# kjyv/FloBaRoID

Measured on AMD Instinct MI355X. Metric: regressor samples/s (fused regressor->Gram pass) + TSQR TFLOP/s, WALK-MAN 31-DOF float-base, higher is better.
Workload: dtype f64

## Files before the change

### flobaroid_amd/csrc/fbr_gram64.h

```cpp
#pragma once
#define FBR_G64_SWZ(c) (2 * ((c) & 15))
#include <algorithm>
#include <type_traits>
#include <utility>

#include "fbr_kinid.h"

struct FbrGram64 {
    int NT = 0;
    int NF = 0;
    int nlev = 0, fb = 0, flev = 0, ntr = 0, maxact = 0, npw = 0, wpb = 8;
    long blk_doubles = 0;
    std::vector<int> trow;
    std::vector<int> slab;
    int nstage = 0, base_stages = 0;
    std::vector<int> stage_lev;
    std::vector<int> lev_begin;
    std::vector<int> pieces;
    std::vector<int> wmeta;
    std::vector<int> slot_tiles;
    std::vector<int> tilecol;
    std::vector<int> fcol_tile, fcol_slot;
    std::vector<int> tile_lo;
    long mfma_per_block = 0;
    long busiest = 0, balanced = 0;
};

static inline bool fbr_gram64_build(const FbrHostModel &hm, const FbrGramProgram &gp, FbrGram64 &g, bool force_tiles = true, bool wide16 = false)
{
    if (gp.T != 1 || (gp.k > 0 && gp.rhs_tiles)) return false;
    g.npw = gp.cfg.segw * gp.cfg.nseg;
    g.wpb = FBR_WPB;
    if (wide16 && g.npw > 10) {
        g.wpb = 2 * FBR_WPB;
        g.npw = 10;
    }
    const int W = g.wpb;
    g.NT = gp.NT;
    g.fb = hm.fb;
    g.nlev = 0;
    std::vector<int> tlo(gp.NT, 0), thi(gp.NT, 0);
    for (int t = 0; t < gp.NT; t++) {
        const FbrTile &tl = gp.tiles[t];
        if (tl.type != 0) return false;
        thi[t] = hm.fb + (int)tl.tpath.size();
        if (tl.friction) {
            int jmin = (int)tl.tpath.size(), jmax = -1;
            for (int sl = 0; sl < FBR_TILE; sl++) {
                if (tl.col[sl] < 0) continue;
                const int jnt = hm.coldesc[tl.col[sl]].joint;
                for (int j = 0; j < (int)tl.tpath.size(); j++)
                    if (tl.tpath[j] == jnt) jmin = std::min(jmin, j), jmax = std::max(jmax, j);
// ... 147 lines not shown
                const int w1 = wave_of[i];
                if (w2 == w1 || cnt[w2] >= g.npw) continue;
                shift(i, w1, -1), shift(i, w2, +1);
                long c1, q1;
                score(c1, q1);
                if (c1 < c0 || (c1 == c0 && q1 < q0)) {
                    wave_of[i] = w2, c0 = c1, q0 = q1, improved = 1;
                } else {
                    shift(i, w2, -1), shift(i, w1, +1);
                }
            }
            for (int k2 = i + 1; k2 < NP; k2++) {
                const int w1 = wave_of[i], w2 = wave_of[k2];
                if (w1 == w2 || (prs[i].lo == prs[k2].lo && prs[i].hi == prs[k2].hi)) continue;
                shift(i, w1, -1), shift(k2, w2, -1), shift(i, w2, +1), shift(k2, w1, +1);
                long c1, q1;
                score(c1, q1);
                if (c1 < c0 || (c1 == c0 && q1 < q0)) {
                    wave_of[i] = w2, wave_of[k2] = w1, c0 = c1, q0 = q1, improved = 1;
                } else {
                    shift(i, w2, -1), shift(k2, w1, -1), shift(i, w1, +1), shift(k2, w2, +1);
                }
            }
        }
    }
    g.busiest = c0;
    g.balanced = 0;
    for (int sg = 0; sg < g.nstage; sg++) {
        int tot = 0;
        for (int lv = g.stage_lev[sg]; lv < g.stage_lev[sg + 1]; lv++)
            for (int w = 0; w < W; w++) tot += wl[w][lv];
        g.balanced += (tot + W - 1) / W;
    }
    g.wmeta.assign((size_t)W * g.npw * 3, -1);
    g.slot_tiles.assign((size_t)2 * W * g.npw * 2, -1);
    g.mfma_per_block = 0;
    for (int w = 0; w < W; w++) {
        std::vector<int> mine;
        for (int i = 0; i < NP; i++)
            if (wave_of[i] == w) mine.push_back(i);
        std::vector<char> done(NP, 0);
        int q = 0;
        for (size_t left = mine.size(); left > 0;) {
            std::vector<int> freq(NTT, 0);
            for (int i : mine)
                if (!done[i]) {
                    freq[prs[i].a]++;
                    if (prs[i].b != prs[i].a) freq[prs[i].b]++;
                }
            int T = 0;
            for (int t = 1; t < NTT; t++)
                if (freq[t] > freq[T]) T = t;
            for (int i : mine) {
                if (done[i] || (prs[i].a != T && prs[i].b != T)) continue;
                const int J = prs[i].a == T ? prs[i].b : prs[i].a;
                const size_t s = (size_t)w * g.npw + q;
                const size_t sr = ((size_t)(w & 7) * (W / 8) + (size_t)(w >> 3)) * g.npw + q;
                g.wmeta[3 * s] = T;
                g.wmeta[3 * s + 1] = J;
                g.wmeta[3 * s + 2] = prs[i].lo | (prs[i].hi << 8);
                const int kind = T >= g.NT ? 1 : 0;
                g.slot_tiles[((size_t)kind * W * g.npw + sr) * 2] = T;
                g.slot_tiles[((size_t)kind * W * g.npw + sr) * 2 + 1] = J;
                g.mfma_per_block += 16L * (prs[i].hi - prs[i].lo);
                done[i] = 1;
                q++;
                left--;
            }
        }
    }
    return true;
}

#define FBR_G64_WORDS 18
#define FBR_G64_FRIC 4
struct FbrGram64Producer {
    int nparts = 1, nslots = 1, step0[FBR_KINWRITE_PARTS] = {0, 0, 0, 0}, nsteps[FBR_KINWRITE_PARTS] = {0, 0, 0, 0};
    std::vector<long long> rel;
    std::vector<int> lcol;
    std::vector<int> steps;
};

static inline bool fbr_gram64_build_producer(const FbrHostModel &hm, const FbrGramProgram &gp, const FbrGram64 &g, FbrGram64Producer &pr)
{
    std::vector<int> tile_of(hm.cols, -1), slot_of(hm.cols, -1);
    for (int t = 0; t < g.NT; t++)
        for (int sl = 0; sl < FBR_TILE; sl++)
            if (gp.tiles[t].col[sl] >= 0 && gp.tiles[t].col[sl] < hm.cols) {
                tile_of[gp.tiles[t].col[sl]] = t;
                slot_of[gp.tiles[t].col[sl]] = sl;
            }
    std::vector<double> lcost(hm.L, 30.0);
    for (int c = 0; c < hm.ninert; c++)
        if (tile_of[c] >= 0) lcost[hm.coldesc[c].link] += 10.0 + (double)(hm.fb + hm.path[hm.coldesc[c].link].size());
    std::vector<FbrKinIdProgram> progs;
    std::vector<std::vector<char>> own;
    try {
        fbr_kinid_build_parts(hm, lcost, FBR_KINWRITE_PARTS, progs, own);
    } catch (const std::exception &) {
        return false;
    }
    pr.nparts = (int)progs.size();
    pr.rel.assign((size_t)pr.nparts * FBR_G64_WORDS * hm.L, 0);
    pr.lcol.assign((size_t)pr.nparts * (10 + FBR_G64_FRIC) * hm.L, -1);
// ... 20 lines not shown
    for (int c = hm.ninert; c < hm.cols; c++) {
        const int t = tile_of[c], sl = slot_of[c], d = hm.coldesc[c].joint, p = (c - hm.ninert) / std::max(hm.n, 1);
        if (t < 0) continue;
        int l = -1;
        for (int x = 0; x < hm.L; x++)
            if (hm.dof[x] == d) l = x;
        if (l < 0 || p >= FBR_G64_FRIC || hm.path[l].empty() || hm.path[l].back() != d) return false;
        const int lv = hm.fb + (int)hm.path[l].size() - 1;
        if (lv < g.tile_lo[t] || g.trow[(size_t)t * g.nlev + lv] < 0) return false;
        const long long tr0 = (long long)g.trow[(size_t)t * g.nlev + g.tile_lo[t]] - g.tile_lo[t];
        if (tr0 < 0) return false;
        for (int pq = 0; pq < pr.nparts; pq++)
            if (own[pq][l]) {
                pr.rel[((size_t)pq * hm.L + l) * FBR_G64_WORDS + 14 + p] = word(tr0, sl);
                pr.lcol[(size_t)pr.nparts * 10 * hm.L + ((size_t)pq * hm.L + l) * FBR_G64_FRIC + p] = c;
            }
    }
    pr.steps.clear();
    pr.nslots = 1;
    for (int pq = 0; pq < pr.nparts; pq++) {
        pr.step0[pq] = (int)(pr.steps.size() / FBR_KINID_STEP);
        pr.nsteps[pq] = progs[pq].nsteps;
        pr.nslots = std::max(pr.nslots, progs[pq].nslots);
        pr.steps.insert(pr.steps.end(), progs[pq].steps.begin(), progs[pq].steps.begin() + (size_t)progs[pq].nsteps * FBR_KINID_STEP);
    }
    return true;
}

#if defined(__HIPCC__) && defined(FBR_KERNELS_GRAM)
struct DevGram64 {
    int NT, nlev, maxact, npieces, nstage;
    long blk_doubles;
    const int *slab, *lev_begin, *pieces, *wmeta, *stage_lev;
};

template <int MAXD, bool HASW>
__global__ __launch_bounds__(64 * FBR_KINWRITE_PARTS, MAXD <= 10 ? 2 : 1) void fbr_kinimg_kernel(DevModel m, DevKinId p, DevKinWrite wr, long S, long blk_doubles,
                                                                              const double *__restrict__ q, const double *__restrict__ dq,
                                                                              const double *__restrict__ ddq, const double *__restrict__ bv,
                                                                              const double *__restrict__ ba, const double *__restrict__ rpy,
                                                                              const double *__restrict__ rhs, const double *__restrict__ wts,
                                                                              double *__restrict__ scratch, double *__restrict__ mom,
                                                                              const double *__restrict__ sign)
{
    extern __shared__ __attribute__((aligned(16))) double smem[];
    const int lane = threadIdx.x & 63, part = __builtin_amdgcn_readfirstlane(threadIdx.x >> 6), nth = blockDim.x, tid = threadIdx.x;
    const int n = m.n, ldn = p.ldn, ldw = m.rows | 1, rows = m.rows;
    double *sq = smem, *sdq = sq + 64 * ldn, *sddq = sdq + 64 * ldn, *sw = sddq + 64 * ldn;
    double *st = sw + (HASW ? 64 * ldw : 0);
    double *scr = scratch + ((long)blockIdx.x * wr.nparts + part) * p.nslots * FBR_LINK_REC * 64 + lane;
    double *mo = mom ? mom + (long)blockIdx.x * (wr.cols + 1) * 64 : nullptr;
    const long Sg = wr.group_samples > 0 ? wr.group_samples : S, bpg = (Sg + 63) >> 6;
    const long nblk = (S / Sg) * bpg;
    const fbr_clong_ptr cdst = (fbr_clong_ptr)(unsigned long)wr.dst;
    const fbr_cint_ptr ccol = (fbr_cint_ptr)(unsigned long)(wr.lcol10 + (long)part * 10 * m.L);
    for (long blk = blockIdx.x; blk < nblk; blk += gridDim.x) {
        const long grp = blk / bpg, lb = blk - grp * bpg;
        const long base = grp * Sg + (lb << 6);
        const int valid = (int)min(64L, Sg - (lb << 6));
        __syncthreads();
        {
            const long off = base * n;
            const int cnt = valid * n;
            int sr = tid / n, dc = tid - sr * n;
            const int ds = nth / n, dd = nth - ds * n;
            for (int i = tid; i < cnt; i += nth) {
// ... 189 lines not shown
        blk[(long)tr * 1024 + (sl >> 5) * 512 + c * 32 + ((sl & 31) ^ FBR_G64_SWZ(c))] = 0.0;
    }
}

__global__ __launch_bounds__(256) void fbr_gram64_mom_reduce_kernel(int P, int nwg, const double *__restrict__ mom, double *__restrict__ G)
{
    __shared__ double part[256];
    const int c = blockIdx.x, t = threadIdx.x;
    double s0 = 0.0, s1 = 0.0, s2 = 0.0, s3 = 0.0;
    int i = t;
    for (; i + 768 < nwg * 64; i += 1024) {
        s0 += mom[((long)(i >> 6) * (P + 1) + c) * 64 + (i & 63)];
        s1 += mom[((long)((i + 256) >> 6) * (P + 1) + c) * 64 + ((i + 256) & 63)];
        s2 += mom[((long)((i + 512) >> 6) * (P + 1) + c) * 64 + ((i + 512) & 63)];
        s3 += mom[((long)((i + 768) >> 6) * (P + 1) + c) * 64 + ((i + 768) & 63)];
    }
    for (; i < nwg * 64; i += 256) s0 += mom[((long)(i >> 6) * (P + 1) + c) * 64 + (i & 63)];
    part[t] = (s0 + s1) + (s2 + s3);
    __syncthreads();
    for (int o = 128; o > 0; o >>= 1) {
        if (t < o) part[t] += part[t + o];
        __syncthreads();
    }
    if (t) return;
    const int Pa = P + 1;
    if (c == P) {
        G[(long)P * Pa + P] += part[0];
    } else {
        G[(long)c * Pa + P] += part[0];
        G[(long)P * Pa + c] += part[0];
    }
}

template <int NPW, int WPB>
__global__ __launch_bounds__(WPB * 64, (NPW <= 10) ? 4 : 2) void fbr_gram64_kernel(DevGram64 g, long nblk, const double *__restrict__ img,
                                                                                  double *__restrict__ partial, int carry)
{
    constexpr int MW = 3 * NPW;
    static_assert(MW <= 64, "a wave's slot table is fetched with one load");
    extern __shared__ __attribute__((aligned(16))) double smem[];
    const int bufd = g.maxact * 512;
    double *buf0 = smem, *buf1 = smem + bufd;
    int *slab = (int *)(smem + 2 * bufd);
    int *levb = slab + g.nlev * g.NT;
    int *pcs = levb + g.nlev + 1;
    int *wm = pcs + 2 * g.npieces;
    int *stl = wm + WPB * MW;
    const int tid = threadIdx.x, lane = tid & 63;
    const int wave = __builtin_amdgcn_readfirstlane(tid >> 6);
    for (int i = tid; i < g.nlev * g.NT; i += WPB * 64) slab[i] = g.slab[i];
    for (int i = tid; i <= g.nlev; i += WPB * 64) levb[i] = g.lev_begin[i];
    for (int i = tid; i < 2 * g.npieces; i += WPB * 64) pcs[i] = g.pieces[i];
    for (int i = tid; i < WPB * MW; i += WPB * 64) wm[i] = g.wmeta[i];
    for (int i = tid; i <= g.nstage; i += WPB * 64) stl[i] = g.stage_lev[i];
    fbr_d4 acc[NPW];
    img += (long)blockIdx.y * nblk * g.blk_doubles;
    double *pp = partial + (((((long)blockIdx.y * gridDim.x + blockIdx.x) * 8 + (wave & 7)) * (WPB / 8) + (wave >> 3)) * NPW) * 256;
    if (carry) {
#pragma unroll
        for (int q = 0; q < NPW; q++) acc[q] = (fbr_d4){pp[q * 256 + lane], pp[q * 256 + 64 + lane], pp[q * 256 + 128 + lane], pp[q * 256 + 192 + lane]};
    } else {
#pragma unroll
        for (int q = 0; q < NPW; q++) acc[q] = (fbr_d4){0.0, 0.0, 0.0, 0.0};
    }
    __syncthreads();
    const int nmine = (int)((nblk - blockIdx.x + gridDim.x - 1) / gridDim.x);
    const long nst = (long)(nmine > 0 ? nmine : 0) * 2 * g.nstage;
    const int svl = stl[lane <= g.nstage ? lane : 0], svp = levb[svl];
    auto dma = [&](int sg, long bh, int par) {
        const long blk = (long)blockIdx.x + (bh >> 1) * gridDim.x;
        const double *src = img + blk * g.blk_doubles + (bh & 1) * 512 + 2 * lane;
        double *buf = par ? buf1 : buf0;
        const int i0 = __builtin_amdgcn_readlane(svp, sg) + wave, i1 = __builtin_amdgcn_readlane(svp, sg + 1);
        const int mine = i0 < i1 ? (i1 - i0 + WPB - 1) / WPB : 0;
        const int il = i0 + (lane < mine ? lane : 0) * WPB;
        const int gxv = mine > 0 ? pcs[2 * il] : 0, lxv = mine > 0 ? pcs[2 * il + 1] : 0;
        for (int j = 0; j < mine; j++) {
            const int gx = __builtin_amdgcn_readlane(gxv, j), lx = __builtin_amdgcn_readlane(lxv, j);
            __builtin_amdgcn_global_load_lds((fbr_glb_ptr)(src + gx), (fbr_lds_ptr)(buf + lx), 16, 0, 0);
        }
    };
    if (nst > 0) dma(0, 0, 0);
    const int li = lane & 15, kk = lane >> 4;
    const int lofs = li * 32, sx = FBR_G64_SWZ(li);
    const int mv = wm[wave * MW + (lane < MW ? lane : 0)];
    const int idxv = (lane < MW && (lane % 3) != 2 && mv >= 0) ? mv : 0;
    const int p0c = lofs | (sx ^ kk);
    int sg = 0;
    long bh = 0;
    for (long st = 0; st < nst; st++) {
        asm volatile("s_waitcnt vmcnt(0)" ::: "memory");
        __syncthreads();
        const int sgn = sg + 1 == g.nstage ? 0 : sg + 1;
        const long bhn = sgn ? bh : bh + 1;
        if (st + 1 < nst) dma(sgn, bhn, (int)((st + 1) & 1));
        const double *buf = (st & 1) ? buf1 : buf0;
        const int lv0 = __builtin_amdgcn_readlane(svl, sg), lv1 = __builtin_amdgcn_readlane(svl, sg + 1);
        sg = sgn;
        bh = bhn;
        for (int lv = lv0; lv < lv1; lv++) {
            const int offv = slab[lv * g.NT + idxv] * 512;
            int curI = -1;
            double a[8] = {0.0, 0.0, 0.0, 0.0, 0.0, 0.0, 0.0, 0.0};
#pragma unroll
            for (int q = 0; q < NPW; q++) {
                const int tI = __builtin_amdgcn_readlane(mv, 3 * q), rg = __builtin_amdgcn_readlane(mv, 3 * q + 2);
                if (tI < 0 || lv < (rg & 0xff) || lv >= (rg >> 8)) continue;
                const double *pb = buf + __builtin_amdgcn_readlane(offv, 3 * q + 1);
                double b[NPW <= 10 ? 4 : 8];
                int p0 = p0c;
                if constexpr (NPW <= 10) asm volatile("" : "+v"(p0));
                if (tI != curI) {
                    const double *pa = buf + __builtin_amdgcn_readlane(offv, 3 * q);
#pragma unroll
                    for (int ks = 0; ks < 8; ks++) a[ks] = pa[p0 ^ (4 * ks)];
                    curI = tI;
                }
                constexpr int KG = NPW <= 10 ? 4 : 8;
#pragma unroll
                for (int k0 = 0; k0 < 8; k0 += KG) {
#pragma unroll
                    for (int ks = k0; ks < k0 + KG; ks++) b[ks - k0] = pb[p0 ^ (4 * ks)];
                    __builtin_amdgcn_sched_barrier(0);
#pragma unroll
                    for (int ks = k0; ks < k0 + KG; ks++) acc[q] = __builtin_amdgcn_mfma_f64_16x16x4f64(a[ks], b[ks - k0], acc[q], 0, 0, 0);
                    __builtin_amdgcn_sched_barrier(0);
                }
            }
        }
    }
#pragma unroll
    for (int q = 0; q < NPW; q++) {
        pp[q * 256 + 0 * 64 + lane] = acc[q][0];
        pp[q * 256 + 1 * 64 + lane] = acc[q][1];
        pp[q * 256 + 2 * 64 + lane] = acc[q][2];
        pp[q * 256 + 3 * 64 + lane] = acc[q][3];
    }
}
#endif
```

### flobaroid_amd/csrc/fbr_gram_api.hip

```cpp
#define FBR_KERNELS_GRAM
#include "fbr_internal.h"

static int get_deal(GramHolder *h, int wpg, GramHolder::Deal *out, bool base_only = false)
{
    const int key = wpg | (base_only ? 1 << 24 : 0);
    auto it = h->deals.find(key);
    if (it != h->deals.end()) {
        *out = it->second;
        return FBR_OK;
    }
    const std::vector<int> n = fbr_gram_deal(h->prog, wpg, base_only);
    std::vector<int2> tab;
    std::vector<int> begin(h->prog.T + 1, 0), given(h->prog.T, 0);
    for (int p = 0; p < h->prog.T; p++) begin[p + 1] = begin[p] + n[p];
    while ((int)tab.size() < begin[h->prog.T])
        for (int p = 0; p < h->prog.T; p++)
            if (given[p] < n[p]) tab.push_back(make_int2(p, given[p]++ | (n[p] << 16)));
    GramHolder::Deal d;
    int rc;
    if ((rc = upload(h->pool, tab, &d.tab))) return rc;
    if ((rc = upload(h->pool, begin, &d.begin))) return rc;
    h->deals[key] = d;
    *out = d;
    return FBR_OK;
// ... 174 lines not shown
    if (num_pairs) *num_pairs = (int32_t)h->prog.pairs.size();
    if (mfma_per_sample) *mfma_per_sample = h->prog.mfma_per_sample;
    if (num_parts) *num_parts = h->prog.T;
    return FBR_OK;
}

static int get_gram64(fbr_model *m, GramHolder *h);

extern "C" int fbr_gram_lane_info(const fbr_model *mc, int32_t k, int64_t num_samples, int64_t info[12])
{
    if (!mc || !info) {
        set_err("null model / info");
        return FBR_E_INVALID;
    }
    fbr_model *m = const_cast<fbr_model *>(mc);
    if (int rc_enter = enter(m)) return rc_enter;
    if (const int wr = pick_gram_reduction(m, num_samples < 0 ? -1 : (long)num_samples); wr >= 0) m = m->rdm[wr].get();
    for (int i = 0; i < 12; i++) info[i] = 0;
    if ((m->hm.rows + 3) / 4 * 4 > 60) return FBR_OK;
    const bool moments = fbr_gram_rhs_moments(m->hm, k, m->opt.gram_rhs_tile != 0);
    GramHolder *h = nullptr;
    int rc = get_gram(m, k, &h, moments);
    if (rc) return rc;
    if (!m->opt.gram_lane || k > 1 || (k == 1 && !moments)) return FBR_OK;
    if ((rc = get_gram64(m, h))) return rc;
    if (h->g64_state != 1) return FBR_OK;
    const FbrGram64 &g = h->g64;
    info[0] = 1;
    info[1] = g.ntr;
    info[2] = g.blk_doubles * (int64_t)sizeof(double);
    info[3] = g.mfma_per_block;
    info[4] = g.nlev;
    info[5] = g.maxact;
    info[6] = (int64_t)((size_t)2 * g.maxact * 512 * sizeof(double) +
                        ((size_t)g.nlev * (g.NT + g.NF) + g.nlev + 1 + g.pieces.size() + g.wmeta.size() + g.stage_lev.size()) * sizeof(int));
    info[7] = g.NT;
    info[8] = g.NF;
    info[9] = g.busiest;
    info[10] = g.balanced;
    info[11] = g.nstage;
    return FBR_OK;
}

__global__ __launch_bounds__(256) void fbr_rtr_kernel(int Pa, const double *__restrict__ R, double *__restrict__ G, int accumulate)
{
    for (long e = (long)blockIdx.x * blockDim.x + threadIdx.x; e < (long)Pa * Pa; e += (long)gridDim.x * blockDim.x) {
        const int i = (int)(e / Pa), j = (int)(e % Pa);
        double acc = 0.0;
        for (int r = 0; r <= min(i, j); r++) acc += R[(long)r * Pa + i] * R[(long)r * Pa + j];
        G[e] = accumulate ? G[e] + acc : acc;
    }
}

static int gram_via_tsqr(fbr_model *m, const fbr_states *st, const double *rhs, int32_t k, const double *w, double *G_out, int32_t out_mem,
                         int32_t accumulate)
{
    const int Pa = m->hm.cols + k;
    const size_t cnt = (size_t)Pa * Pa;
    int rc;
    if ((rc = m->gram_r_tmp.ensure(cnt * sizeof(double)))) return rc;
    double *R = m->gram_r_tmp.as<double>();
    if ((rc = tsqr_impl(m, st, nullptr, 0, rhs, k, w, nullptr, R, FBR_DEVICE, nullptr))) return rc;
    double *G = G_out;
    if (out_mem == FBR_HOST) {
        if ((rc = m->g_tmp.ensure(cnt * sizeof(double)))) return rc;
        G = m->g_tmp.as<double>();
        if (accumulate) HIPCHK(hipMemcpyAsync(G, G_out, cnt * sizeof(double), hipMemcpyHostToDevice, m->stream));
    }
    hipLaunchKernelGGL(fbr_rtr_kernel, dim3(1024), dim3(256), 0, m->stream, Pa, R, G, accumulate ? 1 : 0);
    HIPCHK(hipGetLastError());
    return finish_output(m, G, G_out, cnt, out_mem);
}
static int get_gram64(fbr_model *m, GramHolder *h)
{
    if (h->g64_state) return FBR_OK;
    h->g64_state = -1;
    const FbrHostModel &hm = m->hm;
    if (m->kinid.nsteps <= 0 || !fbr_gram64_build(hm, h->prog, h->g64, m->opt.gram_force_tiles != 0, m->opt.gram_lane_waves >= 16)) return FBR_OK;
    FbrGram64 &g = h->g64;
    const size_t lds = (size_t)2 * g.maxact * 512 * sizeof(double) +
                       ((size_t)g.nlev * (g.NT + g.NF) + g.nlev + 1 + g.pieces.size() + g.wmeta.size() + g.stage_lev.size()) * sizeof(int);
    if (lds > 156 * 1024) return FBR_OK;
    const size_t plds_max = ((size_t)3 * 64 * (std::max(hm.n, 1) | 1) + (size_t)2 * 64 * (hm.rows | 1)) * sizeof(double);
    if (plds_max > 160 * 1024) return FBR_OK;
    if (!fbr_gram64_build_producer(hm, h->prog, g, h->g64p)) return FBR_OK;
    std::vector<int> wgbegin{0, 0};
    int rc;
    if ((rc = upload(h->pool, g.slab, &h->d64_slab)) || (rc = upload(h->pool, g.lev_begin, &h->d64_levb)) || (rc = upload(h->pool, g.pieces, &h->d64_pieces)) ||
        (rc = upload(h->pool, g.wmeta, &h->d64_wmeta)) || (rc = upload(h->pool, h->g64p.lcol, &h->d64_lcol)) ||
        (rc = upload(h->pool, h->g64p.steps, &h->d64_steps)) ||
        (rc = upload(h->pool, g.slot_tiles, &h->d64_slot_tiles)) || (rc = upload(h->pool, g.tilecol, &h->d64_tilecol)) ||
        (rc = upload(h->pool, g.stage_lev, &h->d64_stagelev)))
        return rc;
    h->g64_state = 1;
    return FBR_OK;
}

static long gram64_chunk_blocks(const FbrGram64 &g) { return std::max<long>(1, (long)((size_t)3 * 1024 * 1024 * 1024 / ((size_t)g.blk_doubles * 8))); }

static int gram64_wg_table(GramHolder *h, int wgs, const int **out)
{
    auto it = h->d64_wb.find(wgs);
    if (it == h->d64_wb.end()) {
        std::vector<int> wb{0, wgs};
        const int *dwb = nullptr;
        if (int rc = upload(h->pool, wb, &dwb)) return rc;
        it = h->d64_wb.emplace(wgs, dwb).first;
    }
    *out = it->second;
    return FBR_OK;
}

static int gram64_ensure_images(fbr_model *m, GramHolder *h, long chb)
{
    const FbrGram64 &g = h->g64;
    int rc;
    if (chb <= h->img64_blocks) return FBR_OK;
    for (int b = 0; b < 2; b++) {
        if ((rc = h->img64[b].ensure((size_t)chb * g.blk_doubles * sizeof(double)))) return rc;
        HIPCHK(hipMemsetAsync(h->img64[b].p, 0, h->img64[b].bytes, m->stream));
        std::vector<long long> dst(h->g64p.rel.size(), 0);
        for (size_t i = 0; i < dst.size(); i++)
            if (h->g64p.rel[i]) dst[i] = (long long)(uintptr_t)h->img64[b].p + (h->g64p.rel[i] & ~(1LL << 62));
        if ((rc = h->dst64[b].ensure(dst.size() * sizeof(long long)))) return rc;
        HIPCHK(hipMemcpyAsync(h->dst64[b].p, dst.data(), dst.size() * sizeof(long long), hipMemcpyHostToDevice, m->stream));
        HIPCHK(hipStreamSynchronize(m->stream));
    }
    h->img64_blocks = chb;
    return FBR_OK;
}

static int gram64_pass(fbr_model *m, GramHolder *h, const DevStates &d, const double *drhs, const double *dw, int k, double *G, bool base_only,
                       bool h2d_chunked)
{
    const FbrHostModel &hm = m->hm;
    FbrGram64 &g = h->g64;
    const long S = d.S;
    const int Pa = hm.cols + k;
    int rc;
    const long nblocks = (S + 63) / 64;
    long chb = gram64_chunk_blocks(g);
    if (h2d_chunked) chb = std::min<long>(chb, 7L * m->num_cus);
    if (m->opt.chunk_samples >= 1) chb = std::min(gram64_chunk_blocks(g), std::max<long>(1, ((long)m->opt.chunk_samples + 63) / 64));
    chb = std::min(nblocks, chb);
    if (chb < nblocks && chb > m->num_cus) chb = chb / m->num_cus * m->num_cus;
    if ((rc = gram64_ensure_images(m, h, chb))) return rc;
    const int ldn = std::max(hm.n, 1) | 1, ldw = hm.rows | 1;
    const size_t plds = ((size_t)3 * 64 * ldn + (dw ? (size_t)64 * ldw : 0) + (k ? (size_t)64 * ldw : 0)) * sizeof(double);
    const int pgrid_max = (m->kinid.maxlvl <= 10 ? 2 : 1) * m->num_cus;
    const int pblocks = (int)std::min<long>(chb, (long)pgrid_max);
    const int gwgs = (int)std::min<long>(chb, (long)m->num_cus);
    if ((rc = h->scr64.ensure((size_t)pgrid_max * h->g64p.nparts * std::max(h->g64p.nslots, 1) * FBR_LINK_REC * 64 * sizeof(double)))) return rc;
    if (k) {
        if ((rc = h->mom64.ensure((size_t)pgrid_max * (hm.cols + 1) * 64 * sizeof(double)))) return rc;
        HIPCHK(hipMemsetAsync(h->mom64.p, 0, (size_t)pblocks * (hm.cols + 1) * 64 * sizeof(double), m->stream));
    }
    const int npw = g.npw;
    if ((rc = m->partial.ensure((size_t)m->num_cus * g.wpb * npw * 256 * sizeof(double)))) return rc;
    const size_t glds = (size_t)2 * g.maxact * 512 * sizeof(double) + ((size_t)g.nlev * (g.NT + g.NF) + g.nlev + 1 + g.pieces.size() + g.wmeta.size() + g.stage_lev.size()) * sizeof(int);
    DevKinId kp;
    kp.nsteps = 0;
    kp.maxlvl = m->kinid.maxlvl;
    kp.nslots = h->g64p.nslots;
    kp.ldn = ldn;
    kp.steps = h->d64_steps;
    kp.endflush = m->kinid_endflush;
    DevGram64 dg;
    dg.NT = g.NT + g.NF;
    dg.nlev = g.nlev;
    dg.maxact = g.maxact;
    dg.npieces = (int)g.pieces.size() / 2;
    dg.blk_doubles = g.blk_doubles;
    dg.slab = h->d64_slab;
    dg.lev_begin = h->d64_levb;
    dg.pieces = h->d64_pieces;
    dg.wmeta = h->d64_wmeta;
    dg.nstage = base_only ? g.base_stages : g.nstage;
    dg.stage_lev = h->d64_stagelev;
    typedef void (*g64_fn)(DevGram64, long, const double *, double *, int);
    const g64_fn gk = g.wpb == 16 ? fbr_gram64_kernel<10, 16> : (g.npw == 10 ? fbr_gram64_kernel<10, 8> : fbr_gram64_kernel<FBR_ONE_SEGW * FBR_ONE_NSEG, 8>);
    const int vnpw = g.npw * (g.wpb / 8);
    HIPCHK(hipFuncSetAttribute((const void *)gk, hipFuncAttributeMaxDynamicSharedMemorySize, (int)glds));
    int launches = 0, first_wgs = 0;
    const size_t stage_per = (size_t)3 * hm.n + (hm.floating ? 15 : 0) + (d.sign ? hm.n : 0) + (size_t)hm.rows * k + (dw ? hm.rows : 0);
    if (h2d_chunked) {
        for (int b = 0; b < 2; b++)
            if ((rc = m->st_chunk[b].ensure(std::max<size_t>(1, (size_t)chb * 64 * stage_per) * sizeof(double)))) return rc;
        if (!m->copy) {
            int least = 0, greatest = 0;
            HIPCHK(hipDeviceGetStreamPriorityRange(&least, &greatest));
            HIPCHK(hipStreamCreateWithPriority(&m->copy, hipStreamNonBlocking, greatest));
        }
        HIPCHK(hipEventRecord(m->ev_fork, m->stream));
    }
    struct Staged {
        DevStates dc;
        long o;
        const double *rhs, *w;
    };
    auto stage = [&](long c, Staged &out) -> int {
        const long s0 = c * chb * 64, cs = std::min(chb * 64, S - s0);
        const int b = (int)(c & 1);
        out.dc = d;
        out.o = s0;
        out.rhs = drhs;
        out.w = dw;
        if (!h2d_chunked) return FBR_OK;
        HIPCHK(hipStreamWaitEvent(m->copy, m->ev_pack_rec[b] ? m->ev_pack[b] : m->ev_fork, 0));
        ProfScope ps(m, FBR_PROF_H2D, m->copy);
        double *p = m->st_chunk[b].as<double>();
        auto put = [&](const double *src, size_t per, const double **dst) -> int {
            *dst = nullptr;
            if (!src || per == 0) return FBR_OK;
// ... 97 lines not shown
        if ((rc = gram64_wg_table(h, first_wgs, &dr.wg_begin))) return rc;
        dr.tilecol = h->d64_tilecol;
        hipLaunchKernelGGL(fbr_gram_reduce_kernel, dim3(FBR_WPB * vnpw, 1), dim3(256), 0, m->stream, dr, m->partial.as<double>(), G);
        HIPCHK(hipGetLastError());
        if (g.NF > 0) {
            dr.slot_tiles = h->d64_slot_tiles + (size_t)FBR_WPB * vnpw * 2;
            hipLaunchKernelGGL(fbr_gram_reduce_kernel, dim3(FBR_WPB * vnpw, 1), dim3(256), 0, m->stream, dr, m->partial.as<double>(), G);
            HIPCHK(hipGetLastError());
        }
        if (k) {
            hipLaunchKernelGGL(fbr_gram64_mom_reduce_kernel, dim3(hm.cols + 1), dim3(256), 0, m->stream, hm.cols, pblocks, h->mom64.as<double>(), G);
            HIPCHK(hipGetLastError());
        }
    }
    (void)Pa;
    return FBR_OK;
}

static int gram64_grouped_pass(fbr_model *m, GramHolder *h, const DevStates &d, const double *dw, double *G, int ngroups)
{
    const FbrHostModel &hm = m->hm;
    FbrGram64 &g = h->g64;
    const long S = d.S, Sg = S / ngroups, bpg = (Sg + 63) / 64;
    const int Pa = hm.cols, npw = g.npw;
    int rc;
    const int gpc = (int)std::min<long>(std::min(ngroups, 32768), std::max<long>(1, gram64_chunk_blocks(g) / bpg));
    if ((rc = gram64_ensure_images(m, h, (long)gpc * bpg))) return rc;
    const int wpg = (int)std::max<long>(1, std::min<long>(bpg, (long)m->num_cus / std::min(gpc, ngroups)));
    const int ldn = std::max(hm.n, 1) | 1, ldw = hm.rows | 1;
    const size_t plds = ((size_t)3 * 64 * ldn + (dw ? (size_t)64 * ldw : 0)) * sizeof(double);
    const int pgrid_max = (m->kinid.maxlvl <= 10 ? 2 : 1) * m->num_cus;
    if ((rc = h->scr64.ensure((size_t)pgrid_max * h->g64p.nparts * std::max(h->g64p.nslots, 1) * FBR_LINK_REC * 64 * sizeof(double)))) return rc;
    if ((rc = m->partial.ensure((size_t)gpc * wpg * g.wpb * npw * 256 * sizeof(double)))) return rc;
    const size_t glds = (size_t)2 * g.maxact * 512 * sizeof(double) + ((size_t)g.nlev * (g.NT + g.NF) + g.nlev + 1 + g.pieces.size() + g.wmeta.size() + g.stage_lev.size()) * sizeof(int);
    DevKinId kp;
    kp.nsteps = 0;
    kp.maxlvl = m->kinid.maxlvl;
    kp.nslots = h->g64p.nslots;
    kp.ldn = ldn;
    kp.steps = h->d64_steps;
    kp.endflush = m->kinid_endflush;
    DevGram64 dg;
    dg.NT = g.NT + g.NF;
    dg.nlev = g.nlev;
    dg.maxact = g.maxact;
    dg.npieces = (int)g.pieces.size() / 2;
    dg.blk_doubles = g.blk_doubles;
    dg.slab = h->d64_slab;
    dg.lev_begin = h->d64_levb;
    dg.pieces = h->d64_pieces;
    dg.wmeta = h->d64_wmeta;
    dg.nstage = g.nstage;
    dg.stage_lev = h->d64_stagelev;
    typedef void (*g64_fn)(DevGram64, long, const double *, double *, int);
    const g64_fn gk = g.wpb == 16 ? fbr_gram64_kernel<10, 16> : (g.npw == 10 ? fbr_gram64_kernel<10, 8> : fbr_gram64_kernel<FBR_ONE_SEGW * FBR_ONE_NSEG, 8>);
    const int vnpw = g.npw * (g.wpb / 8);
    HIPCHK(hipFuncSetAttribute((const void *)gk, hipFuncAttributeMaxDynamicSharedMemorySize, (int)glds));
    const int *wgb = nullptr;
    if ((rc = gram64_wg_table(h, wpg, &wgb))) return rc;
    int launches = 0;
    for (int g0 = 0; g0 < ngroups; g0 += gpc, launches++) {
        const int ng = std::min(gpc, ngroups - g0), b = launches & 1;
        const long s0 = (long)g0 * Sg, cs = (long)ng * Sg, nb = (long)ng * bpg;
        DevKinWrite kw;
        kw.lcol10 = h->d64_lcol;
        kw.colrec = nullptr;
        kw.dst = (const long *)h->dst64[b].p;
        kw.ninert = hm.ninert;
        kw.cols = hm.cols;
        kw.k = 0;
        kw.has_w = dw ? 1 : 0;
        kw.flev = g.flev;
        kw.base_only = 0;
        kw.group_samples = Sg;
        kw.nparts = h->g64p.nparts;
        for (int pq = 0; pq < FBR_KINWRITE_PARTS; pq++) {
            kw.part_nsteps[pq] = h->g64p.nsteps[pq];
            kw.part_step0[pq] = h->g64p.step0[pq];
        }
        const int pblocks = (int)std::min<long>(nb, (long)pgrid_max);
        if (Sg & 63) {
            hipLaunchKernelGGL(fbr_gram64_tail_zero_kernel, dim3(16, ng), dim3(256), 0, m->stream, h->img64[b].as<double>(), g.blk_doubles, bpg, g.ntr, (int)(Sg & 63));
            HIPCHK(hipGetLastError());
        }
        {
            ProfScope ps(m, FBR_PROF_PACK);
#define FBR_KINIMG_GLAUNCH2(D, W)                                                                                                                 \
    do {                                                                                                                                         \
// ... 456 lines not shown
```

### flobaroid_amd/csrc/fbr_internal.h

```cpp
#pragma once
#include <hip/hip_runtime.h>
#include <unistd.h>

#include <algorithm>
#include <cstdint>
#include <cstdio>
#include <cstdlib>
#include <cstring>
#include <map>
#include <memory>
#include <numeric>
#include <string>
#include <vector>

#include "../../include/fbr.h"
#include "fbr_options.h"
#include "fbr_kernels.h"
#include "fbr_kinid.h"
#include "fbr_gram64.h"
#include "fbr_tsqr_work.h"

extern thread_local std::string g_fbr_err;
static inline void set_err(const std::string &s) { g_fbr_err = s; }

// ... 49 lines not shown
        p = nullptr;
        bytes = 0;
    }
    template <class T> T *as() { return (T *)p; }
};

template <class T> static inline int upload(std::vector<DevBuf> &pool, const std::vector<T> &v, const T **out)
{
    pool.emplace_back();
    DevBuf &b = pool.back();
    size_t n = std::max<size_t>(v.size(), 1) * sizeof(T);
    int rc = b.ensure(n);
    if (rc) return rc;
    if (!v.empty()) HIPCHK(hipMemcpy(b.p, v.data(), v.size() * sizeof(T), hipMemcpyHostToDevice));
    *out = (const T *)b.p;
    return FBR_OK;
}

struct GramHolder {
    FbrGramProgram prog;
    DevGram dev;
    std::vector<DevBuf> pool;
    DevBuf pimg[2];
    bool moments = false;
    DevBuf mom[2];
    bool mom_clean[2] = {false, false};
    const int *itemcol = nullptr;
    size_t lds_bytes = 0;
    size_t pack_lds_bytes = 0;
    int g64_state = 0;
    FbrGram64 g64;
    FbrGram64Producer g64p;
    const int *d64_slab = nullptr, *d64_levb = nullptr, *d64_pieces = nullptr, *d64_wmeta = nullptr, *d64_lcol = nullptr,
              *d64_steps = nullptr, *d64_slot_tiles = nullptr, *d64_tilecol = nullptr, *d64_stagelev = nullptr;
    DevBuf img64[2], dst64[2], mom64, scr64;
    long img64_blocks = 0;
    std::map<int, const int *> d64_wb;
    struct Deal { const int2 *tab; const int *begin; };
    std::map<int, Deal> deals;
};

struct fbr_model {
    FbrOptions opt;
    FbrHostModel hm;
    DevModel dm;
    int device = 0;
    pid_t pid = 0;
    int num_cus = 256;
    hipStream_t own_stream = nullptr, stream = nullptr;
    hipStream_t side = nullptr;
    hipStream_t copy = nullptr;
    hipEvent_t ev_pack[2] = {nullptr, nullptr}, ev_gram[2] = {nullptr, nullptr}, ev_fork = nullptr, ev_h2d[2] = {nullptr, nullptr};
    hipEvent_t ev_done[2] = {nullptr, nullptr};
    int64_t next_ticket = 0;
    int64_t waited_ticket = -1;
    bool submitting = false;
    bool ev_gram_rec[2] = {false, false};
    bool ev_pack_rec[2] = {false, false};
    DevBuf rec2;
    std::vector<DevBuf> tables;
    std::map<int, std::unique_ptr<GramHolder>> gram;
    DevBuf st_q, st_dq, st_ddq, st_bv, st_ba, st_rpy, st_sign, st_aux, st_aux2, st_x;
    DevBuf rec, partial, out_tmp, g_tmp;
    DevBuf st_chunk[2];
    DevBuf fd[7];
    DevBuf row_flags;
    FbrKinIdProgram kinid;
// ... 139 lines not shown
```

Measured before the change: 76.59 million.

## Add run-based software-pipelined MFMA path for wide gram64 slot tables

Sorts each wave's slot list so that the slots active at every level form one contiguous run, and stores per-level run bounds in LDS. A new RUNS kernel variant walks only the active run. It double-buffers the operand fragments with inline assembly, interleaving ds_read prefetches of the next slot with the MFMAs of the current one and reusing the shared tile when it repeats. The slab offsets are also prescaled at LDS load time. This adds complex hand-written asm with manual waitcnt handling and register pressure, and the path applies only when the run structure is valid for the 8-wave wide shape.

Result: faster. 79.51 million (median of 6 runs) (+3.8%).

```diff
diff --git a/flobaroid_amd/csrc/fbr_gram64.h b/flobaroid_amd/csrc/fbr_gram64.h
--- a/flobaroid_amd/csrc/fbr_gram64.h
+++ b/flobaroid_amd/csrc/fbr_gram64.h
@@ -18,6 +18,7 @@
     std::vector<int> lev_begin;
     std::vector<int> pieces;
     std::vector<int> wmeta;
+    std::vector<int> runs;
     std::vector<int> slot_tiles;
     std::vector<int> tilecol;
     std::vector<int> fcol_tile, fcol_slot;
@@ -231,15 +232,12 @@
             for (int w = 0; w < W; w++) tot += wl[w][lv];
         g.balanced += (tot + W - 1) / W;
     }
-    g.wmeta.assign((size_t)W * g.npw * 3, -1);
-    g.slot_tiles.assign((size_t)2 * W * g.npw * 2, -1);
-    g.mfma_per_block = 0;
+    std::vector<std::vector<int>> slots(W);
     for (int w = 0; w < W; w++) {
         std::vector<int> mine;
         for (int i = 0; i < NP; i++)
             if (wave_of[i] == w) mine.push_back(i);
         std::vector<char> done(NP, 0);
-        int q = 0;
         for (size_t left = mine.size(); left > 0;) {
             std::vector<int> freq(NTT, 0);
             for (int i : mine)
@@ -253,22 +251,68 @@
             for (int i : mine) {
                 if (done[i] || (prs[i].a != T && prs[i].b != T)) continue;
                 const int J = prs[i].a == T ? prs[i].b : prs[i].a;
-                const size_t s = (size_t)w * g.npw + q;
-                const size_t sr = ((size_t)(w & 7) * (W / 8) + (size_t)(w >> 3)) * g.npw + q;
-                g.wmeta[3 * s] = T;
-                g.wmeta[3 * s + 1] = J;
-                g.wmeta[3 * s + 2] = prs[i].lo | (prs[i].hi << 8);
-                const int kind = T >= g.NT ? 1 : 0;
-                g.slot_tiles[((size_t)kind * W * g.npw + sr) * 2] = T;
-                g.slot_tiles[((size_t)kind * W * g.npw + sr) * 2 + 1] = J;
-                g.mfma_per_block += 16L * (prs[i].hi - prs[i].lo);
+                slots[w].insert(slots[w].end(), {T, J, prs[i].lo, prs[i].hi});
                 done[i] = 1;
-                q++;
                 left--;
             }
         }
     }
+    g.runs.clear();
+    if (W == 8 && g.npw > 10) {
+        std::vector<std::vector<int>> sorted(W);
+        std::vector<int> runs((size_t)W * g.nlev, 0);
+        bool ok = true;
+        for (int w = 0; w < W && ok; w++) {
+            const int n = (int)slots[w].size() / 4;
+            std::vector<int> ord(n);
+            for (int q = 0; q < n; q++) ord[q] = q;
+            const int *sw = slots[w].data();
+            std::stable_sort(ord.begin(), ord.end(), [&](int x, int y) {
+                const bool fx = sw[4 * x] >= g.NT, fy = sw[4 * y] >= g.NT;
+                return fx != fy ? fx : sw[4 * x + 3] > sw[4 * y + 3];
+            });
+            for (int q : ord) sorted[w].insert(sorted[w].end(), sw + 4 * q, sw + 4 * q + 4);
+            for (int lv = 0; lv < g.nlev && ok; lv++) {
+                int qa = -1, qb = -1;
+                for (int q = 0; q < n; q++) {
+                    const bool act = sorted[w][4 * q + 2] <= lv && lv < sorted[w][4 * q + 3];
+                    if (act && qa < 0) qa = q;
+                    if (act && qb >= 0) ok = false;
+                    if (!act && qa >= 0 && qb < 0) qb = q;
+                }
+                if (qa < 0) qa = qb = 0;
+                else if (qb < 0) qb = n;
+                runs[(size_t)w * g.nlev + lv] = qa | (qb << 8);
+            }
+        }
+        if (ok) {
+            slots.swap(sorted);
+            g.runs.swap(runs);
+        }
+    }
+    g.wmeta.assign((size_t)W * g.npw * 3, -1);
+    g.slot_tiles.assign((size_t)2 * W * g.npw * 2, -1);
+    g.mfma_per_block = 0;
+    for (int w = 0; w < W; w++)
+        for (int q = 0; q < (int)slots[w].size() / 4; q++) {
+            const int T = slots[w][4 * q], J = slots[w][4 * q + 1], lo = slots[w][4 * q + 2], hi = slots[w][4 * q + 3];
+            const size_t s = (size_t)w * g.npw + q;
+            const size_t sr = ((size_t)(w & 7) * (W / 8) + (size_t)(w >> 3)) * g.npw + q;
+            g.wmeta[3 * s] = T;
+            g.wmeta[3 * s + 1] = J;
+            g.wmeta[3 * s + 2] = lo | (hi << 8);
+            const int kind = T >= g.NT ? 1 : 0;
+            g.slot_tiles[((size_t)kind * W * g.npw + sr) * 2] = T;
+            g.slot_tiles[((size_t)kind * W * g.npw + sr) * 2 + 1] = J;
+            g.mfma_per_block += 16L * (hi - lo);
+        }
     return true;
+}
+
+static inline size_t fbr_gram64_lds_bytes(const FbrGram64 &g)
+{
+    return (size_t)2 * g.maxact * 512 * sizeof(double) +
+           ((size_t)g.nlev * (g.NT + g.NF) + g.nlev + 1 + g.pieces.size() + g.wmeta.size() + g.stage_lev.size() + g.runs.size()) * sizeof(int);
 }
 
 #define FBR_G64_WORDS 18
@@ -355,6 +399,7 @@
     int NT, nlev, maxact, npieces, nstage;
     long blk_doubles;
     const int *slab, *lev_begin, *pieces, *wmeta, *stage_lev;
+    const int *runs;
 };
 
 template <int MAXD, bool HASW>
@@ -610,7 +655,7 @@
     }
 }
 
-template <int NPW, int WPB>
+template <int NPW, int WPB, bool RUNS = false>
 __global__ __launch_bounds__(WPB * 64, (NPW <= 10) ? 4 : 2) void fbr_gram64_kernel(DevGram64 g, long nblk, const double *__restrict__ img,
                                                                                   double *__restrict__ partial, int carry)
 {
@@ -623,13 +668,17 @@
     int *levb = slab + g.nlev * g.NT;
     int *pcs = levb + g.nlev + 1;
     int *wm = pcs + 2 * g.npieces;
-    int *stl = wm + WPB * MW;
+    int *rn = wm + WPB * MW;
+    static_assert(!RUNS || NPW > 10, "the 128-register shapes walk every slot");
+    int *stl = rn + (RUNS ? WPB * g.nlev : 0);
     const int tid = threadIdx.x, lane = tid & 63;
     const int wave = __builtin_amdgcn_readfirstlane(tid >> 6);
-    for (int i = tid; i < g.nlev * g.NT; i += WPB * 64) slab[i] = g.slab[i];
+    for (int i = tid; i < g.nlev * g.NT; i += WPB * 64) slab[i] = g.slab[i] * 512;
     for (int i = tid; i <= g.nlev; i += WPB * 64) levb[i] = g.lev_begin[i];
     for (int i = tid; i < 2 * g.npieces; i += WPB * 64) pcs[i] = g.pieces[i];
     for (int i = tid; i < WPB * MW; i += WPB * 64) wm[i] = g.wmeta[i];
+    if (RUNS)
+        for (int i = tid; i < WPB * g.nlev; i += WPB * 64) rn[i] = g.runs[i];
     for (int i = tid; i <= g.nstage; i += WPB * 64) stl[i] = g.stage_lev[i];
     fbr_d4 acc[NPW];
     img += (long)blockIdx.y * nblk * g.blk_doubles;
@@ -664,6 +713,95 @@
     const int mv = wm[wave * MW + (lane < MW ? lane : 0)];
     const int idxv = (lane < MW && (lane % 3) != 2 && mv >= 0) ? mv : 0;
     const int p0c = lofs | (sx ^ kk);
+    static_assert(!RUNS || MW < 63, "lane 63 holds the run");
+    const int *lk = lane == 63 ? rn + wave * g.nlev : slab + idxv;
+    const int lks = lane == 63 ? 1 : g.NT;
+    const unsigned rlm = [&] {
+        unsigned m = 0;
+#pragma unroll
+        for (int q = 1; q < NPW; q++) m |= (unsigned)(__builtin_amdgcn_readlane(mv, 3 * q) != __builtin_amdgcn_readlane(mv, 3 * q - 3)) << q;
+        return (unsigned)__builtin_amdgcn_readfirstlane((int)m);
+    }();
+    int ko[8];
+#pragma unroll
+    for (int ks = 0; ks < 8; ks++) ko[ks] = (p0c ^ (4 * ks)) * 8;
+    double X[2][8], Y[2][8];
+#pragma unroll
+    for (int ks = 0; ks < 8; ks++) X[0][ks] = X[1][ks] = Y[0][ks] = Y[1][ks] = 0.0;
+    auto run_stage = [&](const double *buf, int lv0, int lv1) {
+        const unsigned bufb = (unsigned)(unsigned long)(fbr_lds_ptr)buf;
+        int offv = lk[lv0 * lks];
+        for (int lv = lv0; lv < lv1; lv++) {
+            const int cur = offv;
+            offv = lk[(lv + 1 < g.nlev ? lv + 1 : lv) * lks];
+            const int run = __builtin_amdgcn_readlane(cur, 63), qa = run & 0xff, qb = run >> 8;
+#define G64_RD(D, S, K, T) "v_add_u32 %[" T "], %[" S "], %[o" #K "]\n\tds_read_b64 %[" D #K "], %[" T "]\n\t"
+#define G64_MF(K) "v_mfma_f64_16x16x4_f64 %[acc], %[xa" #K "], %[xb" #K "], %[acc]\n\t"
+#define G64_MV(K) "v_mov_b64 %[ya" #K "], %[xa" #K "]\n\t"
+#pragma unroll
+            for (int q = 0; q < NPW; q++) {
+                if (q < qa || q >= qb) continue;
+                const int P = q & 1, N = P ^ 1;
+                int t0, t1;
+                if (q == qa) {
+                    const unsigned sa = bufb + (__builtin_amdgcn_readlane(cur, 3 * q) << 3), sb = bufb + (__builtin_amdgcn_readlane(cur, 3 * q + 1) << 3);
+                    asm volatile(G64_RD("xa", "sa", 0, "t0") G64_RD("xa", "sa", 1, "t1") G64_RD("xa", "sa", 2, "t0") G64_RD("xa", "sa", 3, "t1")
+                                 G64_RD("xa", "sa", 4, "t0") G64_RD("xa", "sa", 5, "t1") G64_RD("xa", "sa", 6, "t0") G64_RD("xa", "sa", 7, "t1")
+                                 G64_RD("xb", "sb", 0, "t0") G64_RD("xb", "sb", 1, "t1") G64_RD("xb", "sb", 2, "t0") G64_RD("xb", "sb", 3, "t1")
+                                 G64_RD("xb", "sb", 4, "t0") G64_RD("xb", "sb", 5, "t1") G64_RD("xb", "sb", 6, "t0") G64_RD("xb", "sb", 7, "t1")
+                                 : [t0] "=&v"(t0), [t1] "=&v"(t1),
+                                   [xa0] "+v"(X[P][0]), [xa1] "+v"(X[P][1]), [xa2] "+v"(X[P][2]), [xa3] "+v"(X[P][3]),
+                                   [xa4] "+v"(X[P][4]), [xa5] "+v"(X[P][5]), [xa6] "+v"(X[P][6]), [xa7] "+v"(X[P][7]),
+                                   [xb0] "+v"(Y[P][0]), [xb1] "+v"(Y[P][1]), [xb2] "+v"(Y[P][2]), [xb3] "+v"(Y[P][3]),
+                                   [xb4] "+v"(Y[P][4]), [xb5] "+v"(Y[P][5]), [xb6] "+v"(Y[P][6]), [xb7] "+v"(Y[P][7])
+                                 : [sa] "s"(sa), [sb] "s"(sb),
+                                   [o0] "v"(ko[0]), [o1] "v"(ko[1]), [o2] "v"(ko[2]), [o3] "v"(ko[3]), [o4] "v"(ko[4]), [o5] "v"(ko[5]), [o6] "v"(ko[6]), [o7] "v"(ko[7])
+                                 : "memory");
+                }
+                const int f = __builtin_amdgcn_readfirstlane((q + 1 < qb ? 4 : 0) | ((rlm >> (q + 1)) & 1 ? 8 : 0));
+                const unsigned sna = q + 1 < NPW ? bufb + (__builtin_amdgcn_readlane(cur, 3 * q + 3) << 3) : 0u;
+                const unsigned snb = q + 1 < NPW ? bufb + (__builtin_amdgcn_readlane(cur, 3 * q + 4) << 3) : 0u;
+                asm volatile(
+                    "s_waitcnt lgkmcnt(0)\n\t"
+                    G64_MF(0)
+                    "s_bitcmp0_b32 %[f], 2\n\t"
+                    "s_cbranch_scc1 3f\n\t"
+                    G64_RD("yb", "snb", 0, "t0") G64_RD("yb", "snb", 1, "t1") G64_MF(1)
+                    G64_RD("yb", "snb", 2, "t0") G64_RD("yb", "snb", 3, "t1") G64_MF(2)
+                    G64_RD("yb", "snb", 4, "t0") G64_RD("yb", "snb", 5, "t1") G64_MF(3)
+                    G64_RD("yb", "snb", 6, "t0") G64_RD("yb", "snb", 7, "t1") G64_MF(4)
+                    "s_bitcmp0_b32 %[f], 3\n\t"
+                    "s_cbranch_scc1 2f\n\t"
+                    G64_RD("ya", "sna", 0, "t0") G64_RD("ya", "sna", 1, "t1") G64_RD("ya", "sna", 2, "t0") G64_RD("ya", "sna", 3, "t1") G64_MF(5)
+                    G64_RD("ya", "sna", 4, "t0") G64_RD("ya", "sna", 5, "t1") G64_RD("ya", "sna", 6, "t0") G64_RD("ya", "sna", 7, "t1") G64_MF(6)
+                    G64_MF(7)
+                    "s_branch 9f\n\t"
+                    "2:\n\t"
+                    G64_MV(0) G64_MV(1) G64_MV(2) G64_MV(3) G64_MF(5)
+                    G64_MV(4) G64_MV(5) G64_MV(6) G64_MV(7) G64_MF(6)
+                    G64_MF(7)
+                    "s_branch 9f\n\t"
+                    "3:\n\t"
+                    G64_MF(1) G64_MF(2) G64_MF(3) G64_MF(4) G64_MF(5) G64_MF(6) G64_MF(7)
+                    "9:"
+                    : [acc] "+v"(acc[q]), [t0] "=&v"(t0), [t1] "=&v"(t1),
+                      [xa0] "+v"(X[P][0]), [xa1] "+v"(X[P][1]), [xa2] "+v"(X[P][2]), [xa3] "+v"(X[P][3]),
+                      [xa4] "+v"(X[P][4]), [xa5] "+v"(X[P][5]), [xa6] "+v"(X[P][6]), [xa7] "+v"(X[P][7]),
+                      [xb0] "+v"(Y[P][0]), [xb1] "+v"(Y[P][1]), [xb2] "+v"(Y[P][2]), [xb3] "+v"(Y[P][3]),
+                      [xb4] "+v"(Y[P][4]), [xb5] "+v"(Y[P][5]), [xb6] "+v"(Y[P][6]), [xb7] "+v"(Y[P][7]),
+                      [ya0] "+v"(X[N][0]), [ya1] "+v"(X[N][1]), [ya2] "+v"(X[N][2]), [ya3] "+v"(X[N][3]),
+                      [ya4] "+v"(X[N][4]), [ya5] "+v"(X[N][5]), [ya6] "+v"(X[N][6]), [ya7] "+v"(X[N][7]),
+                      [yb0] "+v"(Y[N][0]), [yb1] "+v"(Y[N][1]), [yb2] "+v"(Y[N][2]), [yb3] "+v"(Y[N][3]),
+                      [yb4] "+v"(Y[N][4]), [yb5] "+v"(Y[N][5]), [yb6] "+v"(Y[N][6]), [yb7] "+v"(Y[N][7])
+                    : [f] "s"(f), [sna] "s"(sna), [snb] "s"(snb),
+                      [o0] "v"(ko[0]), [o1] "v"(ko[1]), [o2] "v"(ko[2]), [o3] "v"(ko[3]), [o4] "v"(ko[4]), [o5] "v"(ko[5]), [o6] "v"(ko[6]), [o7] "v"(ko[7])
+                    : "memory", "scc");
+            }
+#undef G64_RD
+#undef G64_MF
+#undef G64_MV
+        }
+    };
     int sg = 0;
     long bh = 0;
     for (long st = 0; st < nst; st++) {
@@ -676,8 +814,12 @@
         const int lv0 = __builtin_amdgcn_readlane(svl, sg), lv1 = __builtin_amdgcn_readlane(svl, sg + 1);
         sg = sgn;
         bh = bhn;
+        if constexpr (RUNS) {
+            run_stage(buf, lv0, lv1);
+            continue;
+        }
         for (int lv = lv0; lv < lv1; lv++) {
-            const int offv = slab[lv * g.NT + idxv] * 512;
+            const int offv = slab[lv * g.NT + idxv];
             int curI = -1;
             double a[8] = {0.0, 0.0, 0.0, 0.0, 0.0, 0.0, 0.0, 0.0};
 #pragma unroll
@@ -707,6 +849,7 @@
             }
         }
     }
+    if constexpr (RUNS) asm volatile("s_nop 7\n\ts_nop 7\n\ts_nop 7" ::: "memory");
 #pragma unroll
     for (int q = 0; q < NPW; q++) {
         pp[q * 256 + 0 * 64 + lane] = acc[q][0];
diff --git a/flobaroid_amd/csrc/fbr_gram_api.hip b/flobaroid_amd/csrc/fbr_gram_api.hip
--- a/flobaroid_amd/csrc/fbr_gram_api.hip
+++ b/flobaroid_amd/csrc/fbr_gram_api.hip
@@ -230,8 +230,7 @@
     info[3] = g.mfma_per_block;
     info[4] = g.nlev;
     info[5] = g.maxact;
-    info[6] = (int64_t)((size_t)2 * g.maxact * 512 * sizeof(double) +
-                        ((size_t)g.nlev * (g.NT + g.NF) + g.nlev + 1 + g.pieces.size() + g.wmeta.size() + g.stage_lev.size()) * sizeof(int));
+    info[6] = (int64_t)fbr_gram64_lds_bytes(g);
     info[7] = g.NT;
     info[8] = g.NF;
     info[9] = g.busiest;
@@ -276,9 +275,7 @@
     const FbrHostModel &hm = m->hm;
     if (m->kinid.nsteps <= 0 || !fbr_gram64_build(hm, h->prog, h->g64, m->opt.gram_force_tiles != 0, m->opt.gram_lane_waves >= 16)) return FBR_OK;
     FbrGram64 &g = h->g64;
-    const size_t lds = (size_t)2 * g.maxact * 512 * sizeof(double) +
-                       ((size_t)g.nlev * (g.NT + g.NF) + g.nlev + 1 + g.pieces.size() + g.wmeta.size() + g.stage_lev.size()) * sizeof(int);
-    if (lds > 156 * 1024) return FBR_OK;
+    if (fbr_gram64_lds_bytes(g) > 156 * 1024) return FBR_OK;
     const size_t plds_max = ((size_t)3 * 64 * (std::max(hm.n, 1) | 1) + (size_t)2 * 64 * (hm.rows | 1)) * sizeof(double);
     if (plds_max > 160 * 1024) return FBR_OK;
     if (!fbr_gram64_build_producer(hm, h->prog, g, h->g64p)) return FBR_OK;
@@ -288,7 +285,7 @@
         (rc = upload(h->pool, g.wmeta, &h->d64_wmeta)) || (rc = upload(h->pool, h->g64p.lcol, &h->d64_lcol)) ||
         (rc = upload(h->pool, h->g64p.steps, &h->d64_steps)) ||
         (rc = upload(h->pool, g.slot_tiles, &h->d64_slot_tiles)) || (rc = upload(h->pool, g.tilecol, &h->d64_tilecol)) ||
-        (rc = upload(h->pool, g.stage_lev, &h->d64_stagelev)))
+        (rc = upload(h->pool, g.stage_lev, &h->d64_stagelev)) || (!g.runs.empty() && (rc = upload(h->pool, g.runs, &h->d64_runs))))
         return rc;
     h->g64_state = 1;
     return FBR_OK;
@@ -355,7 +352,7 @@
     }
     const int npw = g.npw;
     if ((rc = m->partial.ensure((size_t)m->num_cus * g.wpb * npw * 256 * sizeof(double)))) return rc;
-    const size_t glds = (size_t)2 * g.maxact * 512 * sizeof(double) + ((size_t)g.nlev * (g.NT + g.NF) + g.nlev + 1 + g.pieces.size() + g.wmeta.size() + g.stage_lev.size()) * sizeof(int);
+    const size_t glds = fbr_gram64_lds_bytes(g);
     DevKinId kp;
     kp.nsteps = 0;
     kp.maxlvl = m->kinid.maxlvl;
@@ -375,8 +372,11 @@
     dg.wmeta = h->d64_wmeta;
     dg.nstage = base_only ? g.base_stages : g.nstage;
     dg.stage_lev = h->d64_stagelev;
+    dg.runs = g.runs.empty() ? nullptr : h->d64_runs;
     typedef void (*g64_fn)(DevGram64, long, const double *, double *, int);
-    const g64_fn gk = g.wpb == 16 ? fbr_gram64_kernel<10, 16> : (g.npw == 10 ? fbr_gram64_kernel<10, 8> : fbr_gram64_kernel<FBR_ONE_SEGW * FBR_ONE_NSEG, 8>);
+    const g64_fn gk = g.wpb == 16 ? fbr_gram64_kernel<10, 16>
+                      : g.npw == 10   ? fbr_gram64_kernel<10, 8>
+                      : g.runs.empty() ? fbr_gram64_kernel<FBR_ONE_SEGW * FBR_ONE_NSEG, 8> : fbr_gram64_kernel<FBR_ONE_SEGW * FBR_ONE_NSEG, 8, true>;
     const int vnpw = g.npw * (g.wpb / 8);
     HIPCHK(hipFuncSetAttribute((const void *)gk, hipFuncAttributeMaxDynamicSharedMemorySize, (int)glds));
     int launches = 0, first_wgs = 0;
@@ -540,7 +540,7 @@
     const int pgrid_max = (m->kinid.maxlvl <= 10 ? 2 : 1) * m->num_cus;
     if ((rc = h->scr64.ensure((size_t)pgrid_max * h->g64p.nparts * std::max(h->g64p.nslots, 1) * FBR_LINK_REC * 64 * sizeof(double)))) return rc;
     if ((rc = m->partial.ensure((size_t)gpc * wpg * g.wpb * npw * 256 * sizeof(double)))) return rc;
-    const size_t glds = (size_t)2 * g.maxact * 512 * sizeof(double) + ((size_t)g.nlev * (g.NT + g.NF) + g.nlev + 1 + g.pieces.size() + g.wmeta.size() + g.stage_lev.size()) * sizeof(int);
+    const size_t glds = fbr_gram64_lds_bytes(g);
     DevKinId kp;
     kp.nsteps = 0;
     kp.maxlvl = m->kinid.maxlvl;
@@ -560,8 +560,11 @@
     dg.wmeta = h->d64_wmeta;
     dg.nstage = g.nstage;
     dg.stage_lev = h->d64_stagelev;
+    dg.runs = g.runs.empty() ? nullptr : h->d64_runs;
     typedef void (*g64_fn)(DevGram64, long, const double *, double *, int);
-    const g64_fn gk = g.wpb == 16 ? fbr_gram64_kernel<10, 16> : (g.npw == 10 ? fbr_gram64_kernel<10, 8> : fbr_gram64_kernel<FBR_ONE_SEGW * FBR_ONE_NSEG, 8>);
+    const g64_fn gk = g.wpb == 16 ? fbr_gram64_kernel<10, 16>
+                      : g.npw == 10   ? fbr_gram64_kernel<10, 8>
+                      : g.runs.empty() ? fbr_gram64_kernel<FBR_ONE_SEGW * FBR_ONE_NSEG, 8> : fbr_gram64_kernel<FBR_ONE_SEGW * FBR_ONE_NSEG, 8, true>;
     const int vnpw = g.npw * (g.wpb / 8);
     HIPCHK(hipFuncSetAttribute((const void *)gk, hipFuncAttributeMaxDynamicSharedMemorySize, (int)glds));
     const int *wgb = nullptr;
diff --git a/flobaroid_amd/csrc/fbr_internal.h b/flobaroid_amd/csrc/fbr_internal.h
--- a/flobaroid_amd/csrc/fbr_internal.h
+++ b/flobaroid_amd/csrc/fbr_internal.h
@@ -105,7 +105,8 @@
     FbrGram64 g64;
     FbrGram64Producer g64p;
     const int *d64_slab = nullptr, *d64_levb = nullptr, *d64_pieces = nullptr, *d64_wmeta = nullptr, *d64_lcol = nullptr,
-              *d64_steps = nullptr, *d64_slot_tiles = nullptr, *d64_tilecol = nullptr, *d64_stagelev = nullptr;
+              *d64_steps = nullptr, *d64_slot_tiles = nullptr, *d64_tilecol = nullptr, *d64_stagelev = nullptr,
+              *d64_runs = nullptr;
     DevBuf img64[2], dst64[2], mom64, scr64;
     long img64_blocks = 0;
     std::map<int, const int *> d64_wb;
```
